# yycho0108/qpwcnet

Hardware: AMD Instinct MI355X
Metric: image-pairs/sec at 256x512 fp32 (higher is better)
Workload: dtype f32; 1 GPU; BASELINE configs[1]: full 6-level PWC-Net (qpwcnet build_flower) inference, batch 8 per GPU, 256x512 fp32, channels_last, d=4 cost volume + WarpV2; global_batch=8, batch_per_gpu=8, parallelism=dp1 (pairs sharded, RCCL all-gather of the 6 per-level EPE), hipgraph=True

## Files before the change

### qpwcnet_amd/csrc/encoder.hip

```cpp
#include "common.h"
#include "launch.h"

namespace qpwc {

__device__ __forceinline__ float enc_mishf(float x) {
    const float e = __builtin_amdgcn_exp2f(fminf(x, 20.0f) * 1.4426950408889634f);
    const float t = e * (e + 2.0f);
    const float m = x * (t * __builtin_amdgcn_rcpf(t + 2.0f));
    return m;
}

typedef float f32x4e __attribute__((ext_vector_type(4)));

__device__ __forceinline__ float2 ld2(const float* p) { return *reinterpret_cast<const float2*>(p); }
__device__ __forceinline__ float2 ld2(const __half* p) { return __half22float2(*reinterpret_cast<const __half2*>(p)); }
__device__ __forceinline__ void st4q(float* p, float4 v) { *reinterpret_cast<float4*>(p) = v; }
__device__ __forceinline__ void st4q(__half* p, float4 v) {
    __half2 lo = __floats2half2_rn(v.x, v.y), hi = __floats2half2_rn(v.z, v.w);
    uint2 u;
    u.x = *reinterpret_cast<unsigned*>(&lo);
    u.y = *reinterpret_cast<unsigned*>(&hi);
    *reinterpret_cast<uint2*>(p) = u;
}

// ... 42 lines not shown
                                                              const float* __restrict__ weight,
                                                              const float* __restrict__ bias,
                                                              float* __restrict__ out, int H, int W,
                                                              int pad_h, int pad_w, int tiles_x, int tiles_y,
                                                              int groups_x) {
    constexpr int NQ = C / 4;
    constexpr int NFT = C / 16;
    constexpr int NKC = C / 16;
    constexpr int NLD = (kEcNH * NQ + 255) / 256;
    constexpr int NBUF = NT > 1 ? 2 : 1;
    __shared__ __attribute__((aligned(16))) float in_s[NBUF * kEcNH * C];
    const int tid0 = threadIdx.x;
    const int wave = __builtin_amdgcn_readfirstlane(tid0 >> 6);
    const int lane = tid0 & 63, n0 = lane & 15, g0 = lane >> 4;
    const int grp = xcd_swizzle(blockIdx.x, gridDim.x);
    const int gx0 = grp % groups_x, ty = (grp / groups_x) % tiles_y, b = grp / (groups_x * tiles_y);
    const int tx0 = gx0 * NT;
    const int Y0 = ty * kEcTH;
    const float* xb = x + (int64_t)b * H * W * C;
    const int Ho = H + pad_h, Wo = W + pad_w;
    float* ob = out + (int64_t)b * Ho * Wo * C;

    auto stage_load = [&](int tid, int tx, float4 (&v)[NLD]) {
        const int X0 = tx * kEcTW;
#pragma unroll
        for (int it = 0; it < NLD; ++it) {
            const int idx = tid + 256 * it;
            const int hp = idx / NQ, q = idx - hp * NQ;
            const int hy = hp / kEcHW, hx = hp - hy * kEcHW;
            const int gy = Y0 - 1 + hy, gx = X0 - 1 + hx;
            v[it] = (idx < kEcNH * NQ && gy >= 0 && gy < H && gx >= 0 && gx < W)
                        ? *reinterpret_cast<const float4*>(xb + ((int64_t)gy * W + gx) * C + 4 * q)
                        : make_float4(0.f, 0.f, 0.f, 0.f);
        }
    };
    auto stage_write = [&](int tid, int buf, const float4 (&v)[NLD]) {
#pragma unroll
        for (int it = 0; it < NLD; ++it) {
            const int idx = tid + 256 * it;
            const int hp = idx / NQ, q = idx - hp * NQ;
            if (idx < kEcNH * NQ)
                *reinterpret_cast<float4*>(in_s + buf * (kEcNH * C) + hp * C + 4 * ec_slot<C>(q, hp)) = v[it];
        }
    };
#ifdef QPWC_ENC_STAMP
    const bool census_on = tid0 == 0 && blockIdx.x < 4096;
    long long* census_p = g_enc_census + (blockIdx.x < 4096 ? blockIdx.x : 0) * 6;
    if (census_on)
        census_p[5] = (long long)(unsigned)__builtin_amdgcn_s_getreg((4) | (0 << 6) | (31 << 11)) |
                      ((long long)(unsigned)__builtin_amdgcn_s_getreg((20) | (0 << 6) | (31 << 11)) << 32);
#endif
    ENC_CENSUS(0);
    float4 st[NLD];
    stage_load(tid0, tx0, st);
#ifdef QPWC_ENC_STAMP
    asm volatile("s_waitcnt vmcnt(0)" ::: "memory");
#endif
    ENC_CENSUS(1);
    stage_write(tid0, 0, st);
    __syncthreads();
    ENC_CENSUS(2);

#pragma unroll 1
    for (int t = 0; t < NT; ++t) {
        const int tx = tx0 + t;
        if (tx >= tiles_x) break;
        const bool more = t + 1 < NT && tx + 1 < tiles_x;

        const int X0 = tx * kEcTW;
        const float* tile_s = in_s + (t & (NBUF - 1)) * (kEcNH * C);
        const float* wt = weight;
        int n = n0, g = g0, tid = tid0;
        if (NT > 1) asm volatile("" : "+r"(wt), "+v"(n), "+v"(g), "+v"(tid));
        if (more) stage_load(tid, tx + 1, st);
#pragma unroll
        for (int ft = 0; ft < NFT; ++ft) {
            f32x4e wld[9][NKC];
#pragma unroll
            for (int k = 0; k < 9; ++k)
#pragma unroll
                for (int kc = 0; kc < NKC; ++kc)
                    wld[k][kc] = *reinterpret_cast<const f32x4e*>(wt + ((int64_t)k * C + 16 * ft + n) * C + 16 * kc + 4 * g);
            f32x4e acc[2];
            acc[0] = f32x4e{0.f, 0.f, 0.f, 0.f};
            acc[1] = f32x4e{0.f, 0.f, 0.f, 0.f};
#pragma unroll
            for (int ky = 0; ky < 3; ++ky)
#pragma unroll
                for (int kx = 0; kx < 3; ++kx)
#pragma unroll
                    for (int kc = 0; kc < NKC; ++kc) {
                        f32x4e bv[2];
#pragma unroll
                        for (int m = 0; m < 2; ++m) {
                            const int hp = (2 * wave + m + ky) * kEcHW + n + kx;
                            const int q = 4 * kc + g;
                            const int slot = ec_slot<C>(q, hp);
                            bv[m] = *reinterpret_cast<const f32x4e*>(tile_s + hp * C + 4 * slot);
                        }
#pragma unroll
                        for (int tt = 0; tt < 4; ++tt)
#pragma unroll
                            for (int m = 0; m < 2; ++m)
                                acc[m] = __builtin_amdgcn_mfma_f32_16x16x4f32(wld[ky * 3 + kx][kc][tt], bv[m][tt], acc[m], 0, 0, 0);
                    }
            if (ft == NFT - 1) ENC_CENSUS(3);
            const float4 bq = *reinterpret_cast<const float4*>(bias + 16 * ft + 4 * g);
#pragma unroll
            for (int m = 0; m < 2; ++m) {
                const int gy = Y0 + 2 * wave + m, gx = X0 + n;
                if (gy < H && gx < W)
                    *reinterpret_cast<float4*>(ob + ((int64_t)gy * Wo + gx) * C + 16 * ft + 4 * g) =
                        make_float4(enc_mishf(acc[m][0] + bq.x), enc_mishf(acc[m][1] + bq.y),
                                    enc_mishf(acc[m][2] + bq.z), enc_mishf(acc[m][3] + bq.w));
            }
        }
        if (pad_w > 0 && X0 + kEcTW >= W) {
            for (int i = tid; i < kEcTH * pad_w * NQ; i += 256) {
                const int q = i % NQ, r = i / NQ, col = r % pad_w, row = r / pad_w;
                const int gy = Y0 + row;
                if (gy < H) *reinterpret_cast<float4*>(ob + ((int64_t)gy * Wo + W + col) * C + 4 * q) = make_float4(0.f, 0.f, 0.f, 0.f);
            }
        }
        if (pad_h > 0 && Y0 + kEcTH >= H) {
            const int x_end = (X0 + kEcTW >= W) ? Wo : X0 + kEcTW;
            for (int i = tid; i < pad_h * (x_end - X0) * NQ; i += 256) {
                const int q = i % NQ, r = i / NQ, col = r % (x_end - X0), row = r / (x_end - X0);
                *reinterpret_cast<float4*>(ob + ((int64_t)(H + row) * Wo + X0 + col) * C + 4 * q) = make_float4(0.f, 0.f, 0.f, 0.f);
            }
        }
        ENC_CENSUS(4);
        if (more) {
            stage_write(tid, (t + 1) & (NBUF - 1), st);
            __syncthreads();
        }
    }
}

constexpr int kEwSlots = 5;
constexpr unsigned kEwOob = 0x80000000u;

template <int C, int TH>
struct EwShape {
    static constexpr int NKB = C / 32;
    static constexpr int NS = 9 * NKB;
    static constexpr int NH = (TH + 2) * kEcHW;
    static constexpr int NHI = (NH * 8 + 255) / 256;
    static constexpr int HBLK = 4 * NHI * 1024;
    static constexpr int WBASE = 2 * HBLK;
    static constexpr int LDS = WBASE + 4 * kEwSlots * 2048;
    static_assert(NKB % 2 == 0, "the K-loop walks pairs of 32-channel blocks");
};

__device__ __forceinline__ void ew_wait_vm(int n) {
    switch (n) {
#define EW_W(k) case k: asm volatile("s_waitcnt vmcnt(" #k ")" ::: "memory"); break;
        EW_W(1) EW_W(2) EW_W(3) EW_W(4) EW_W(5) EW_W(6) EW_W(7) EW_W(8) EW_W(9) EW_W(10) EW_W(11) EW_W(12)
#undef EW_W
        default: asm volatile("s_waitcnt vmcnt(0)" ::: "memory"); break;
    }
}

__device__ __forceinline__ void ew_dma16(__amdgpu_buffer_rsrc_t r, char* lds, unsigned voff, int soff) {
#ifdef __HIP_DEVICE_COMPILE__
    typedef __attribute__((address_space(3))) void* lds_ptr_t;
    __builtin_amdgcn_raw_ptr_buffer_load_lds(r, (lds_ptr_t)lds, 16, voff, soff, 0, 0);
#endif
}

__device__ __forceinline__ void ew_pin_agpr(f32x4e& v) {
#ifdef __HIP_DEVICE_COMPILE__
    asm volatile("" : "+a"(v));
#endif
}

template <int C, int TH>
__global__ __launch_bounds__(256, (2 * EwShape<C, TH>::LDS <= 160 * 1024) ? 2 : 1) void conv3x3_mish_ring_kernel(
    const float* __restrict__ x, const float* __restrict__ weight, const float* __restrict__ bias,
    float* __restrict__ out, int H, int W, int pad_h, int pad_w, int tiles_x, int tiles_y, int n_tiles) {
    using S = EwShape<C, TH>;
    __shared__ __attribute__((aligned(1024))) char smem[S::LDS];
    const int tid = threadIdx.x;
    const int wave = __builtin_amdgcn_readfirstlane(tid >> 6);
    const int lane = tid & 63, n = lane & 15, g = lane >> 4;
    const int slice = blockIdx.x / n_tiles;
    const int tile = xcd_swizzle(blockIdx.x % n_tiles, n_tiles);
    const int tx = tile % tiles_x, ty = (tile / tiles_x) % tiles_y, b = tile / (tiles_x * tiles_y);
    const int X0 = tx * kEcTW, Y0 = ty * TH;
    const int fo = 64 * slice + 16 * wave;
    const __amdgpu_buffer_rsrc_t rx = __builtin_amdgcn_make_buffer_rsrc(
        const_cast<float*>(x) + (int64_t)b * H * W * C, 0, H * W * C * 4, 0x00020000);
    const __amdgpu_buffer_rsrc_t rw = __builtin_amdgcn_make_buffer_rsrc(const_cast<float*>(weight), 0, 9 * C * C * 4, 0x00020000);

    unsigned hoff[S::NHI];
#pragma unroll
    for (int j = 0; j < S::NHI; ++j) {
        const int i = (wave * S::NHI + j) * 64 + lane;
        const int hp = i >> 3, q = (i & 7) ^ (hp & 7);
        const int hy = hp / kEcHW, hx = hp - hy * kEcHW;
        const int gy = Y0 - 1 + hy, gx = X0 - 1 + hx;
        hoff[j] = (hp < S::NH && gy >= 0 && gy < H && gx >= 0 && gx < W) ? (unsigned)(((gy * W + gx) * C + 4 * q) * 4) : kEwOob;
    }
    const unsigned woff = (unsigned)(((fo + n) * C + 4 * g) * 4);
    auto issue_h = [&](int kb) __attribute__((always_inline)) {
#pragma unroll
        for (int j = 0; j < S::NHI; ++j)
            ew_dma16(rx, smem + (kb & 1) * S::HBLK + (wave * S::NHI + j) * 1024, hoff[j], kb * 128);
    };
    auto issue_w = [&](int s) __attribute__((always_inline)) {
        const int sc = s < S::NS ? s : S::NS - 1;
        const int kb = sc / 9, tap = sc - 9 * kb;
        char* dst = smem + S::WBASE + ((s % kEwSlots) * 4 + wave) * 2048;
#pragma unroll
        for (int kc = 0; kc < 2; ++kc)
            ew_dma16(rw, dst + kc * 1024, woff, (tap * C * C + 32 * kb + 16 * kc) * 4);
    };
    f32x4e wa[2][2], pb[2][2][TH];
    auto read = [&](int s, int buf) __attribute__((always_inline)) {
        const int kb = s / 9, tap = s - 9 * kb, ky = tap / 3, kx = tap - 3 * ky;
        const char* ws = smem + S::WBASE + ((s % kEwSlots) * 4 + wave) * 2048 + lane * 16;
        const char* hs = smem + (kb & 1) * S::HBLK;
#pragma unroll
        for (int kc = 0; kc < 2; ++kc) {
            wa[buf][kc] = *reinterpret_cast<const f32x4e*>(ws + kc * 1024);
#pragma unroll
            for (int m = 0; m < TH; ++m) {
                const int hp = (m + ky) * kEcHW + n + kx;
                pb[buf][kc][m] = *reinterpret_cast<const f32x4e*>(hs + hp * 128 + 16 * ((4 * kc + g) ^ (hp & 7)));
            }
        }
    };
    f32x4e acc[TH];
#pragma unroll
    for (int m = 0; m < TH; ++m) {
        acc[m] = f32x4e{0.f, 0.f, 0.f, 0.f};
        ew_pin_agpr(acc[m]);
    }

    issue_h(0);
#pragma unroll
    for (int s = 0; s < kEwSlots - 1; ++s) issue_w(s);
    ew_wait_vm(2 * (kEwSlots - 2));
    __builtin_amdgcn_s_barrier();
    read(0, 0);

    auto pair = [&](int p, const bool LAST) __attribute__((always_inline)) {
#pragma unroll
        for (int t = 0; t < 18; ++t) {
            const int s = 18 * p + t;
            const bool more = !(LAST && t == 17);
            if (more) {
                const int tb = t % 9;
                const bool h_young = tb >= 1 && tb <= kEwSlots - 2 && !(LAST && t >= 9);
                ew_wait_vm(2 * (kEwSlots - 3) + (h_young ? S::NHI : 0));
                if (tb == 8) {
                    asm volatile("s_waitcnt lgkmcnt(0)" ::: "memory");
                    __builtin_amdgcn_s_barrier();
                }
            }
            issue_w(s + kEwSlots - 1);
            if (t == 0) issue_h(2 * p + 1);
            if (t == 9 && !LAST) issue_h(2 * p + 2);
            if (more) read(s + 1, (t + 1) & 1);
            __builtin_amdgcn_sched_barrier(0);
#pragma unroll
            for (int kc = 0; kc < 2; ++kc)
#pragma unroll
                for (int tt = 0; tt < 4; ++tt)
#pragma unroll
                    for (int m = 0; m < TH; ++m)
                        acc[m] = __builtin_amdgcn_mfma_f32_16x16x4f32(wa[t & 1][kc][tt], pb[t & 1][kc][m][tt], acc[m], 0, 0, 0);
#pragma unroll
            for (int m = 0; m < TH; ++m) ew_pin_agpr(acc[m]);
            __builtin_amdgcn_sched_barrier(0);
        }
    };
#pragma unroll 1
    for (int p = 0; p < S::NKB / 2 - 1; ++p) pair(p, false);
    pair(S::NKB / 2 - 1, true);
    asm volatile("s_waitcnt vmcnt(0)" ::: "memory");

    const int Ho = H + pad_h, Wo = W + pad_w;
    float* ob = out + (int64_t)b * Ho * Wo * C;
    const float4 bq = *reinterpret_cast<const float4*>(bias + fo + 4 * g);
#pragma unroll
    for (int m = 0; m < TH; ++m) {
        const int gy = Y0 + m, gx = X0 + n;
        if (gy < H && gx < W)
            *reinterpret_cast<float4*>(ob + ((int64_t)gy * Wo + gx) * C + fo + 4 * g) =
                make_float4(enc_mishf(acc[m][0] + bq.x), enc_mishf(acc[m][1] + bq.y),
                            enc_mishf(acc[m][2] + bq.z), enc_mishf(acc[m][3] + bq.w));
    }
    if (pad_w > 0 && X0 + kEcTW >= W) {
        for (int i = tid; i < TH * pad_w * 16; i += 256) {
            const int q = i & 15, r = i >> 4, col = r % pad_w, row = r / pad_w;
            const int gy = Y0 + row;
            if (gy < H) *reinterpret_cast<float4*>(ob + ((int64_t)gy * Wo + W + col) * C + 64 * slice + 4 * q) = make_float4(0.f, 0.f, 0.f, 0.f);
        }
    }
    if (pad_h > 0 && Y0 + TH >= H) {
        const int x_end = (X0 + kEcTW >= W) ? Wo : X0 + kEcTW;
        for (int i = tid; i < pad_h * (x_end - X0) * 16; i += 256) {
            const int q = i & 15, r = i >> 4, col = r % (x_end - X0), row = r / (x_end - X0);
            *reinterpret_cast<float4*>(ob + ((int64_t)(H + row) * Wo + X0 + col) * C + 64 * slice + 4 * q) = make_float4(0.f, 0.f, 0.f, 0.f);
        }
    }
}

template <int C, int TH>
static int conv3x3_mish_ring_launch(const void* x, const void* weight, const void* bias, void* out, int B, int H,
// ... 712 lines not shown
    } else {
        constexpr int NP = (kFcIH * kFcIW * 3 + 255) / 256;
        float2 pv[NP];
#pragma unroll
        for (int it = 0; it < NP; ++it) {
            const int idx = tid + 256 * it;
            const int row = idx / (kFcIW * 3), e = idx - row * (kFcIW * 3);
            const int gy = 2 * Y0 + row, gx = 2 * X0 + e / 3;
            pv[it] = make_float2(0.f, 0.f);
            if (idx < kFcIH * kFcIW * 3 && gy < H && gx < W) pv[it] = ld2(xb + ((int64_t)gy * W + 2 * X0) * 6 + 2 * e);
        }
#pragma unroll
        for (int it = 0; it < NP; ++it) {
            const int idx = tid + 256 * it;
            const int row = idx / (kFcIW * 3), e = idx - row * (kFcIW * 3);
            if (idx < kFcIH * kFcIW * 3) *reinterpret_cast<float2*>(in_s + row * (kFcIW * 6) + 2 * e) = pv[it];
        }
    }
    float wv[9];
#pragma unroll
    for (int k = 0; k < 9; ++k) wv[k] = weight[(k * 16 + n) * 4 + g];
    const float4 bq = *reinterpret_cast<const float4*>(bias + 4 * g);
    __syncthreads();

    const int f = wave >> 1;
    T* ob = out + (int64_t)(f * B + b) * Ho * Wo * 16;
    f32x4e acc[kFcTR];
#pragma unroll
    for (int r = 0; r < kFcTR; ++r) acc[r] = f32x4e{0.f, 0.f, 0.f, 0.f};
    float vb[2][kFcTR];
    auto read_tap = [&](float (&v)[kFcTR], int k) __attribute__((always_inline)) {
        const int ky = k / 3, kx = k - 3 * ky;
#pragma unroll
        for (int r = 0; r < kFcTR; ++r) {
            const int oy = kFcTR * (wave & 1) + r;
            v[r] = in_s[((2 * oy + ky) * kFcIW + 2 * n + kx) * 6 + 3 * f + (g < 3 ? g : 2)];
        }
    };
    read_tap(vb[0], 0);
#pragma unroll
    for (int k = 0; k < 9; ++k) {
        if (k + 1 < 9) read_tap(vb[(k + 1) & 1], k + 1);
        __builtin_amdgcn_sched_barrier(0);
#pragma unroll
        for (int r = 0; r < kFcTR; ++r)
            acc[r] = __builtin_amdgcn_mfma_f32_16x16x4f32(wv[k], g < 3 ? vb[k & 1][r] : 0.0f, acc[r], 0, 0, 0);
        __builtin_amdgcn_sched_barrier(0);
    }
#pragma unroll
    for (int r = 0; r < kFcTR; ++r) {
        const int gy = Y0 + kFcTR * (wave & 1) + r, gx = X0 + n;
        if (gy < Ho && gx < Wo)
            st4q(ob + ((int64_t)gy * Wo + gx) * 16 + 4 * g,
                 make_float4(enc_mishf(acc[r][0] + bq.x), enc_mishf(acc[r][1] + bq.y), enc_mishf(acc[r][2] + bq.z),
                             enc_mishf(acc[r][3] + bq.w)));
    }
}

int first_conv_mish_launch(const void* x, const void* weight, const void* bias, void* out, int B, int H, int W,
                           int layout, int dtype, hipStream_t s) {
    const int tiles_x = (W / 2 + kEcTW - 1) / kEcTW, tiles_y = (H / 2 + kFcTH - 1) / kFcTH;
    const int64_t nblk = (int64_t)tiles_x * tiles_y * B;
    if (nblk > INT32_MAX) {
        set_error("first_conv_mish: too many tiles");
        return QPWC_E_SHAPE;
    }
    if (dtype == QPWC_F32)
        hipLaunchKernelGGL(first_conv_mish_kernel<float>, dim3((unsigned)nblk), dim3(256), 0, s, (const float*)x,
                           (const float*)weight, (const float*)bias, (float*)out, B, H, W, tiles_x, tiles_y,
                           layout == QPWC_NCHW ? 1 : 0);
    else
        hipLaunchKernelGGL(first_conv_mish_kernel<__half>, dim3((unsigned)nblk), dim3(256), 0, s, (const __half*)x,
                           (const float*)weight, (const float*)bias, (__half*)out, B, H, W, tiles_x, tiles_y,
                           layout == QPWC_NCHW ? 1 : 0);
    return check_launch("first_conv_mish_kernel");
}

constexpr int kS2IH = 2 * kEcTH + 1;
constexpr int kS2PW = kEcTW + 1;

__global__ __launch_bounds__(256, 4) void conv3x3s2_mish_kernel(const float* __restrict__ x,
                                                                const float* __restrict__ weight,
                                                                const float* __restrict__ bias,
                                                                float* __restrict__ out, int H, int W,
                                                                int tiles_x, int tiles_y) {
    constexpr int CI = 16, CO = 32;
    __shared__ __attribute__((aligned(16))) float in_s[2 * kS2IH * kS2PW * CI];
    const int tid = threadIdx.x;
    const int wave = __builtin_amdgcn_readfirstlane(tid >> 6);
    const int lane = tid & 63, n = lane & 15, g = lane >> 4;
    const int tile = xcd_swizzle(blockIdx.x, gridDim.x);
    const int tx = tile % tiles_x, ty = (tile / tiles_x) % tiles_y, b = tile / (tiles_x * tiles_y);
    const int X0 = tx * kEcTW, Y0 = ty * kEcTH;
    const int Hp = H + 1, Wp = W + 1, Ho = H / 2, Wo = W / 2;
    const float* xb = x + (int64_t)b * Hp * Wp * CI;
    for (int idx = tid; idx < kS2IH * 33 * 4; idx += 256) {
        const int q = idx & 3, pxl = idx >> 2;
        const int row = pxl / 33, col = pxl - row * 33;
        const int gy = 2 * Y0 + row, gx = 2 * X0 + col;
        float4 v = make_float4(0.f, 0.f, 0.f, 0.f);
        if (gy < Hp && gx < Wp) v = *reinterpret_cast<const float4*>(xb + ((int64_t)gy * Wp + gx) * CI + 4 * q);
        const int pix = ((col & 1) * kS2IH + row) * kS2PW + (col >> 1);
        *reinterpret_cast<float4*>(in_s + pix * CI + 4 * ec_slot<CI>(q, pix)) = v;
    }
    f32x4e wv[9][2];
#pragma unroll
    for (int k = 0; k < 9; ++k)
#pragma unroll
        for (int ft = 0; ft < 2; ++ft)
            wv[k][ft] = *reinterpret_cast<const f32x4e*>(weight + ((int64_t)k * CO + 16 * ft + n) * CI + 4 * g);
    __syncthreads();

    f32x4e acc[2][2];
#pragma unroll
    for (int m = 0; m < 2; ++m)
#pragma unroll
        for (int ft = 0; ft < 2; ++ft) acc[m][ft] = f32x4e{0.f, 0.f, 0.f, 0.f};
#pragma unroll
    for (int ky = 0; ky < 3; ++ky)
#pragma unroll
        for (int kx = 0; kx < 3; ++kx) {
            f32x4e bv[2];
#pragma unroll
            for (int m = 0; m < 2; ++m) {
                const int row = 2 * (2 * wave + m) + ky;
                const int par = kx & 1, pc = n + (kx >> 1);
                const int pix = (par * kS2IH + row) * kS2PW + pc;
                bv[m] = *reinterpret_cast<const f32x4e*>(in_s + pix * CI + 4 * ec_slot<CI>(g, pix));
            }
#pragma unroll
            for (int t = 0; t < 4; ++t)
#pragma unroll
                for (int m = 0; m < 2; ++m)
#pragma unroll
                    for (int ft = 0; ft < 2; ++ft)
                        acc[m][ft] = __builtin_amdgcn_mfma_f32_16x16x4f32(wv[ky * 3 + kx][ft][t], bv[m][t], acc[m][ft], 0, 0, 0);
        }
    float* ob = out + (int64_t)b * Ho * Wo * CO;
    const float4 bq2[2] = {*reinterpret_cast<const float4*>(bias + 4 * g), *reinterpret_cast<const float4*>(bias + 16 + 4 * g)};
#pragma unroll
    for (int ft = 0; ft < 2; ++ft) {
        const float4 bq = bq2[ft];
#pragma unroll
        for (int m = 0; m < 2; ++m) {
            const int gy = Y0 + 2 * wave + m, gx = X0 + n;
            if (gy < Ho && gx < Wo)
                *reinterpret_cast<float4*>(ob + ((int64_t)gy * Wo + gx) * CO + 16 * ft + 4 * g) =
                    make_float4(enc_mishf(acc[m][ft][0] + bq.x), enc_mishf(acc[m][ft][1] + bq.y),
                                enc_mishf(acc[m][ft][2] + bq.z), enc_mishf(acc[m][ft][3] + bq.w));
        }
    }
}

template <int CI, int TH>
__global__ __launch_bounds__(256, (2 * (2 * TH + 1) * (kEcTW + 1) * CI * 4 > 80 * 1024) ? 1 : 2) void conv3x3s2_mish_wide_kernel(const float* __restrict__ x,
                                                                     const float* __restrict__ weight,
                                                                     const float* __restrict__ bias,
                                                                     float* __restrict__ out, int H, int W,
                                                                     int tiles_x, int tiles_y, int n_tiles) {
    constexpr int CO = 2 * CI, NQ = CI / 4, NKB = CI / 32;
    constexpr int IH = 2 * TH + 1, PW = kEcTW + 1;
    constexpr int NPX = IH * 33;
    constexpr int NST = (NPX * NQ + 255) / 256;
    __shared__ __attribute__((aligned(16))) float in_s[2 * IH * PW * CI];
    const int tid = threadIdx.x;
    const int wave = __builtin_amdgcn_readfirstlane(tid >> 6);
    const int lane = tid & 63, n = lane & 15, g = lane >> 4;
    const int slice = blockIdx.x / n_tiles;
    const int tile = xcd_swizzle(blockIdx.x % n_tiles, n_tiles);
    const int tx = tile % tiles_x, ty = (tile / tiles_x) % tiles_y, b = tile / (tiles_x * tiles_y);
    const int X0 = tx * kEcTW, Y0 = ty * TH;
    const int Hp = H + 1, Wp = W + 1, Ho = H / 2, Wo = W / 2;
    const int fo = 64 * slice + 16 * wave;
    const float* xb = x + (int64_t)b * Hp * Wp * CI;
    auto slot = [](int q, int pix) { return CI == 32 ? (q ^ ((pix >> 1) & 7)) : (q ^ (pix & 15)); };
    constexpr int kChunk = NST;
#pragma unroll
    for (int base = 0; base < NST; base += kChunk) {
        float4 st[kChunk];
#pragma unroll
        for (int i = 0; i < kChunk; ++i) {
            const int idx = tid + 256 * (base + i);
            const int pxl = idx / NQ, q = idx - pxl * NQ;
            const int row = pxl / 33, col = pxl - row * 33;
            const int gy = 2 * Y0 + row, gx = 2 * X0 + col;
            st[i] = (base + i < NST && idx < NPX * NQ && gy < Hp && gx < Wp)
                        ? *reinterpret_cast<const float4*>(xb + ((int64_t)gy * Wp + gx) * CI + 4 * q)
                        : make_float4(0.f, 0.f, 0.f, 0.f);
        }
#pragma unroll
        for (int i = 0; i < kChunk; ++i) {
            const int idx = tid + 256 * (base + i);
            const int pxl = idx / NQ, q = idx - pxl * NQ;
            const int row = pxl / 33, col = pxl - row * 33;
            const int pix = ((col & 1) * IH + row) * PW + (col >> 1);
            if (base + i < NST && idx < NPX * NQ) *reinterpret_cast<float4*>(in_s + pix * CI + 4 * slot(q, pix)) = st[i];
        }
    }
    f32x4e acc[TH];
#pragma unroll
    for (int m = 0; m < TH; ++m) acc[m] = f32x4e{0.f, 0.f, 0.f, 0.f};
    f32x4e wv[9][2], wn[9][2];
    auto load_w = [&](f32x4e (&w)[9][2], int kb) {
#pragma unroll
        for (int k = 0; k < 9; ++k)
#pragma unroll
            for (int kc = 0; kc < 2; ++kc)
                w[k][kc] = *reinterpret_cast<const f32x4e*>(weight + ((int64_t)k * CO + fo + n) * CI + 32 * kb + 16 * kc + 4 * g);
    };
    load_w(wv, 0);
    __syncthreads();
    auto block = [&](f32x4e (&wv)[9][2], int kb) __attribute__((always_inline)) {
#pragma unroll
        for (int ky = 0; ky < 3; ++ky)
#pragma unroll
            for (int kx = 0; kx < 3; ++kx)
#pragma unroll
                for (int kc = 0; kc < 2; ++kc) {
                    f32x4e bv[TH];
#pragma unroll
                    for (int m = 0; m < TH; ++m) {
                        const int pix = ((kx & 1) * IH + 2 * m + ky) * PW + n + (kx >> 1);
                        bv[m] = *reinterpret_cast<const f32x4e*>(in_s + pix * CI + 4 * slot(8 * kb + 4 * kc + g, pix));
                    }
#pragma unroll
                    for (int t = 0; t < 4; ++t)
#pragma unroll
                        for (int m = 0; m < TH; ++m)
                            acc[m] = __builtin_amdgcn_mfma_f32_16x16x4f32(wv[ky * 3 + kx][kc][t], bv[m][t], acc[m], 0, 0, 0);
                }
    };
#if QPWC_W_NEXT_ALWAYS
    {
        int kb = 0;
#pragma unroll 1
        for (; kb + 1 < NKB; kb += 2) {
            load_w(wn, kb + 1);
            __builtin_amdgcn_sched_barrier(0);
            block(wv, kb);
            load_w(wv, kb + 2 < NKB ? kb + 2 : kb);
            __builtin_amdgcn_sched_barrier(0);
            block(wn, kb + 1);
        }
        if (kb < NKB) block(wv, kb);
    }
#else
#pragma unroll 1
    for (int kb = 0; kb < NKB; ++kb) {
        if (kb + 1 < NKB) load_w(wn, kb + 1);
        block(wv, kb);
#pragma unroll
        for (int k = 0; k < 9; ++k)
#pragma unroll
            for (int kc = 0; kc < 2; ++kc) wv[k][kc] = wn[k][kc];
    }
#endif
    float* ob = out + (int64_t)b * Ho * Wo * CO;
    const float4 bq = *reinterpret_cast<const float4*>(bias + fo + 4 * g);
#pragma unroll
    for (int m = 0; m < TH; ++m) {
        const int gy = Y0 + m, gx = X0 + n;
        if (gy < Ho && gx < Wo)
            *reinterpret_cast<float4*>(ob + ((int64_t)gy * Wo + gx) * CO + fo + 4 * g) =
                make_float4(enc_mishf(acc[m][0] + bq.x), enc_mishf(acc[m][1] + bq.y),
                            enc_mishf(acc[m][2] + bq.z), enc_mishf(acc[m][3] + bq.w));
    }
}

template <int CI, int TH>
static int conv3x3s2_mish_wide_launch(const void* x, const void* weight, const void* bias, void* out, int B,
                                      int H, int W, hipStream_t s) {
    const int tiles_x = (W / 2 + kEcTW - 1) / kEcTW, tiles_y = (H / 2 + TH - 1) / TH;
    const int64_t n_tiles = (int64_t)tiles_x * tiles_y * B;
    const int slices = 2 * CI / 64;
    if (n_tiles * slices > INT32_MAX) {
        set_error("conv3x3s2_mish: too many tiles");
        return QPWC_E_SHAPE;
    }
    hipLaunchKernelGGL((conv3x3s2_mish_wide_kernel<CI, TH>), dim3((unsigned)(n_tiles * slices)), dim3(256), 0, s,
                       (const float*)x, (const float*)weight, (const float*)bias, (float*)out, H, W, tiles_x, tiles_y,
                       (int)n_tiles);
    return check_launch("conv3x3s2_mish_wide_kernel");
}

int conv3x3s2_mish_any_launch(const void* x, const void* weight, const void* bias, void* out, int B, int H, int W,
                              int CI, hipStream_t s);

int conv3x3s2_mish_launch(const void* x, const void* weight, const void* bias, void* out, int B, int H, int W,
                          hipStream_t s) {
    const int tiles_x = (W / 2 + kEcTW - 1) / kEcTW, tiles_y = (H / 2 + kEcTH - 1) / kEcTH;
    const int64_t nblk = (int64_t)tiles_x * tiles_y * B;
    if (nblk > INT32_MAX) {
        set_error("conv3x3s2_mish: too many tiles");
        return QPWC_E_SHAPE;
    }
    hipLaunchKernelGGL(conv3x3s2_mish_kernel, dim3((unsigned)nblk), dim3(256), 0, s, (const float*)x,
                       (const float*)weight, (const float*)bias, (float*)out, H, W, tiles_x, tiles_y);
    return check_launch("conv3x3s2_mish_kernel");
}

int conv3x3s2_mish_any_launch(const void* x, const void* weight, const void* bias, void* out, int B, int H, int W,
                              int CI, hipStream_t s) {
    switch (CI) {
        case 16: return conv3x3s2_mish_launch(x, weight, bias, out, B, H, W, s);
        case 32: return conv3x3s2_mish_wide_launch<32, 4>(x, weight, bias, out, B, H, W, s);
        case 64: return conv3x3s2_mish_wide_launch<64, 2>(x, weight, bias, out, B, H, W, s);
        case 128: return conv3x3s2_mish_wide_launch<128, 2>(x, weight, bias, out, B, H, W, s);
        default: set_error("conv3x3s2_mish: C_in=%d not in {16,32,64,128}", CI); return QPWC_E_SHAPE;
    }
}

template <int CI, int TH>
__global__ __launch_bounds__(256) void conv3x3s2_mish_f16_kernel(const __half* __restrict__ x,
                                                                const __half* __restrict__ weight,
                                                                const float* __restrict__ bias,
                                                                __half* __restrict__ out, int H, int W, int tiles_x,
                                                                int tiles_y, int n_tiles) {
    constexpr int CO = 2 * CI;
    constexpr int CP = CI < 32 ? 32 : CI;
    constexpr int NQ = CP / 8, NQG = CI / 8, NKB = CP / 32;
    constexpr int IH = 2 * TH + 1, PW = kEcTW + 1;
    constexpr int NB = CO / 16;
    constexpr int WB = NB < 4 ? NB : 4, WR = 4 / WB;
    constexpr int RW = TH / WR;
    constexpr int NCH = IH * (2 * kEcTW + 1) * NQ;
    constexpr int NST = (NCH + 255) / 256;
    __shared__ __attribute__((aligned(16))) __half in_s[2 * IH * PW * CP];
    const int tid = threadIdx.x;
    const int wave = __builtin_amdgcn_readfirstlane(tid >> 6);
    const int lane = tid & 63, n = lane & 15, g = lane >> 4;
    const int slice = blockIdx.x / n_tiles;
    const int tile = xcd_swizzle(blockIdx.x % n_tiles, n_tiles);
    const int tx = tile % tiles_x, ty = (tile / tiles_x) % tiles_y, b = tile / (tiles_x * tiles_y);
    const int X0 = tx * kEcTW, Y0 = ty * TH;
    const int Hp = H + 1, Wp = W + 1, Ho = H / 2, Wo = W / 2;
    const __half* xb = x + (int64_t)b * Hp * Wp * CI;
    {
        uint4 st[NST];
#pragma unroll
        for (int it = 0; it < NST; ++it) {
            const int idx = tid + 256 * it;
            const int q = idx % NQ, pc = idx / NQ;
            const int row = pc / (2 * kEcTW + 1), col = pc - row * (2 * kEcTW + 1);
            const int gy = 2 * Y0 + row, gx = 2 * X0 + col;
            st[it] = (idx < NCH && q < NQG && gy < Hp && gx < Wp)
                         ? *reinterpret_cast<const uint4*>(xb + ((int64_t)gy * Wp + gx) * CI + 8 * q)
                         : make_uint4(0u, 0u, 0u, 0u);
        }
#pragma unroll
        for (int it = 0; it < NST; ++it) {
            const int idx = tid + 256 * it;
            const int q = idx % NQ, pc = idx / NQ;
            const int row = pc / (2 * kEcTW + 1), col = pc - row * (2 * kEcTW + 1);
            const int hp = ((col & 1) * IH + row) * PW + (col >> 1);
            if (idx < NCH) *reinterpret_cast<uint4*>(in_s + hp * CP + 8 * f16_slot<CP>(q, hp)) = st[it];
        }
    }
    const int blk = WB == 4 ? 4 * slice + wave : (wave % WB);
    const int r0 = WB == 4 ? 0 : (wave / WB) * RW;
    const int fo = 16 * blk;
    f32x4e acc[RW];
#pragma unroll
    for (int r = 0; r < RW; ++r) acc[r] = f32x4e{0.f, 0.f, 0.f, 0.f};
    const bool kvalid = 8 * g < CI;
    f16x8e wv[9], wn[9];
    auto load_w = [&](f16x8e (&w)[9], int kb) {
#pragma unroll
        for (int tap = 0; tap < 9; ++tap) {
            w[tap] = f16x8e{0, 0, 0, 0, 0, 0, 0, 0};
            if (kvalid) w[tap] = *reinterpret_cast<const f16x8e*>(weight + ((int64_t)tap * CO + fo + n) * CI + 32 * kb + 8 * g);
        }
    };
    load_w(wv, 0);
    __syncthreads();
    auto block = [&](f16x8e (&wv)[9], int kb) __attribute__((always_inline)) {
#pragma unroll
        for (int tap = 0; tap < 9; ++tap) {
            const int ky = tap / 3, kx = tap - 3 * ky;
#pragma unroll
            for (int r = 0; r < RW; ++r) {
                const int hp = ((kx & 1) * IH + 2 * (r0 + r) + ky) * PW + n + (kx >> 1);
                const f16x8e bv = *reinterpret_cast<const f16x8e*>(in_s + hp * CP + 8 * f16_slot<CP>(4 * kb + g, hp));
                acc[r] = __builtin_amdgcn_mfma_f32_16x16x32_f16(wv[tap], bv, acc[r], 0, 0, 0);
            }
        }
    };
#if QPWC_W_NEXT_ALWAYS_F16
    {
        int kb = 0;
#pragma unroll 1
        for (; kb + 1 < NKB; kb += 2) {
            load_w(wn, kb + 1);
            __builtin_amdgcn_sched_barrier(0);
            block(wv, kb);
            load_w(wv, kb + 2 < NKB ? kb + 2 : kb);
            __builtin_amdgcn_sched_barrier(0);
            block(wn, kb + 1);
        }
        if (kb < NKB) block(wv, kb);
    }
#else
#pragma unroll 1
    for (int kb = 0; kb < NKB; ++kb) {
        if (kb + 1 < NKB) load_w(wn, kb + 1);
        block(wv, kb);
#pragma unroll
        for (int tap = 0; tap < 9; ++tap) wv[tap] = wn[tap];
    }
#endif
    __half* ob = out + (int64_t)b * Ho * Wo * CO;
    const float4 bq = *reinterpret_cast<const float4*>(bias + fo + 4 * g);
#pragma unroll
    for (int r = 0; r < RW; ++r) {
        const int gy = Y0 + r0 + r, gx = X0 + n;
        if (gy < Ho && gx < Wo)
            st4q(ob + ((int64_t)gy * Wo + gx) * CO + fo + 4 * g,
                 make_float4(enc_mishf(acc[r][0] + bq.x), enc_mishf(acc[r][1] + bq.y), enc_mishf(acc[r][2] + bq.z),
                             enc_mishf(acc[r][3] + bq.w)));
    }
}

template <int CI, int TH>
static int conv3x3s2_mish_f16_launch_t(const void* x, const void* weight, const void* bias, void* out, int B, int H,
                                       int W, hipStream_t s) {
    constexpr int NSL = (2 * CI / 16) < 4 ? 1 : (2 * CI / 16) / 4;
    const int tiles_x = (W / 2 + kEcTW - 1) / kEcTW, tiles_y = (H / 2 + TH - 1) / TH;
    const int64_t n_tiles = (int64_t)tiles_x * tiles_y * B;
    if (n_tiles * NSL > INT32_MAX) {
        set_error("conv3x3s2_mish_f16: too many tiles");
        return QPWC_E_SHAPE;
    }
    hipLaunchKernelGGL((conv3x3s2_mish_f16_kernel<CI, TH>), dim3((unsigned)(n_tiles * NSL)), dim3(256), 0, s,
                       (const __half*)x, (const __half*)weight, (const float*)bias, (__half*)out, H, W, tiles_x,
                       tiles_y, (int)n_tiles);
    return check_launch("conv3x3s2_mish_f16_kernel");
}

int conv3x3s2_mish_f16_launch(const void* x, const void* weight, const void* bias, void* out, int B, int H, int W,
                              int CI, hipStream_t s) {
    switch (CI) {
        case 16: return conv3x3s2_mish_f16_launch_t<16, 8>(x, weight, bias, out, B, H, W, s);
        case 32: return conv3x3s2_mish_f16_launch_t<32, 8>(x, weight, bias, out, B, H, W, s);
        case 64: return conv3x3s2_mish_f16_launch_t<64, 4>(x, weight, bias, out, B, H, W, s);
        case 128: return conv3x3s2_mish_f16_launch_t<128, 2>(x, weight, bias, out, B, H, W, s);
        default: set_error("conv3x3s2_mish_f16: C_in=%d not in {16,32,64,128}", CI); return QPWC_E_SHAPE;
    }
}

int conv3x3_mish_launch(const void* x, const void* weight, const void* bias, void* out, int B, int H, int W,
                        int C, int pad_h, int pad_w, hipStream_t s) {
    const int tiles_x = (W + kEcTW - 1) / kEcTW, tiles_y = (H + kEcTH - 1) / kEcTH;
    constexpr int NT = QPWC_ENC_NT;
    const int groups_x = (tiles_x + NT - 1) / NT;
    const int64_t nblk = (int64_t)groups_x * tiles_y * B;
    if (nblk > INT32_MAX) {
        set_error("conv3x3_mish: too many tiles");
        return QPWC_E_SHAPE;
    }
    const dim3 grid((unsigned)nblk);
    if (C == 16)
// ... 27 lines not shown
```

Measured before the change: 7304 pairs/s.

## Stream strided conv halo and weights through async LDS DMA ring

Rewrites the stride-2 3x3 conv+Mish encoder kernel for C_in 32/64/128. Halo tiles are now loaded one 32-channel block at a time into double-buffered LDS through buffer_load-to-LDS DMA. Per-tap weights stream through a WS-slot LDS ring, using counted vmcnt waits and barriers so loads overlap the MFMA work. This replaces the old approach of loading the whole halo and holding all 9x2 weight vectors per block in registers. It aims to cut register pressure and exposed load latency, at the cost of more barriers, fragile wait-count bookkeeping, and a new per-tile buffer-size limit.

```diff
diff --git a/qpwcnet_amd/csrc/encoder.hip b/qpwcnet_amd/csrc/encoder.hip
--- a/qpwcnet_amd/csrc/encoder.hip
+++ b/qpwcnet_amd/csrc/encoder.hip
@@ -218,10 +218,12 @@
     static_assert(NKB % 2 == 0, "the K-loop walks pairs of 32-channel blocks");
 };
 
+constexpr int kEwMaxWait = 16;
 __device__ __forceinline__ void ew_wait_vm(int n) {
     switch (n) {
 #define EW_W(k) case k: asm volatile("s_waitcnt vmcnt(" #k ")" ::: "memory"); break;
         EW_W(1) EW_W(2) EW_W(3) EW_W(4) EW_W(5) EW_W(6) EW_W(7) EW_W(8) EW_W(9) EW_W(10) EW_W(11) EW_W(12)
+        EW_W(13) EW_W(14) EW_W(15) EW_W(16)
 #undef EW_W
         default: asm volatile("s_waitcnt vmcnt(0)" ::: "memory"); break;
     }
@@ -1240,17 +1242,40 @@
     }
 }
 
-template <int CI, int TH>
-__global__ __launch_bounds__(256, (2 * (2 * TH + 1) * (kEcTW + 1) * CI * 4 > 80 * 1024) ? 1 : 2) void conv3x3s2_mish_wide_kernel(const float* __restrict__ x,
-                                                                     const float* __restrict__ weight,
-                                                                     const float* __restrict__ bias,
-                                                                     float* __restrict__ out, int H, int W,
-                                                                     int tiles_x, int tiles_y, int n_tiles) {
-    constexpr int CO = 2 * CI, NQ = CI / 4, NKB = CI / 32;
-    constexpr int IH = 2 * TH + 1, PW = kEcTW + 1;
-    constexpr int NPX = IH * 33;
-    constexpr int NST = (NPX * NQ + 255) / 256;
-    __shared__ __attribute__((aligned(16))) float in_s[2 * IH * PW * CI];
+#ifndef QPWC_S2R_TH32
+#define QPWC_S2R_TH32 4
+#define QPWC_S2R_WS32 5
+#endif
+#ifndef QPWC_S2R_TH64
+#define QPWC_S2R_TH64 2
+#define QPWC_S2R_WS64 4
+#endif
+#ifndef QPWC_S2R_TH128
+#define QPWC_S2R_TH128 2
+#define QPWC_S2R_WS128 4
+#endif
+template <int CI, int TH, int WS>
+struct S2rShape {
+    static constexpr int NKB = CI / 32;
+    static constexpr int NS = 9 * NKB;
+    static constexpr int IH = 2 * TH + 1, PW = kEcTW + 1;
+    static constexpr int NP = 2 * IH * PW;
+    static constexpr int NHI = (NP * 8 + 255) / 256;
+    static constexpr int HBLK = 4 * NHI * 1024;
+    static constexpr int WBASE = (NKB > 1 ? 2 : 1) * HBLK;
+    static constexpr int LDS = WBASE + 4 * WS * 2048;
+    static_assert(NKB == 1 || NKB % 2 == 0, "the K-loop walks one block or pairs of 32-channel blocks");
+    static_assert(WS >= 4 && WS <= 9, "W(s + 1) must be older than a younger request, and the halo older than the next block's first weights");
+    static_assert(2 * (WS - 2) <= kEwMaxWait && 2 * (WS - 3) + NHI <= kEwMaxWait, "every wait is a counted one");
+};
+
+template <int CI, int TH, int WS>
+__global__ __launch_bounds__(256, (2 * S2rShape<CI, TH, WS>::LDS <= 160 * 1024) ? 2 : 1) void conv3x3s2_mish_ring_kernel(
+    const float* __restrict__ x, const float* __restrict__ weight, const float* __restrict__ bias,
+    float* __restrict__ out, int H, int W, int tiles_x, int tiles_y, int n_tiles) {
+    using S = S2rShape<CI, TH, WS>;
+    constexpr int CO = 2 * CI;
+    __shared__ __attribute__((aligned(1024))) char smem[S::LDS];
     const int tid = threadIdx.x;
     const int wave = __builtin_amdgcn_readfirstlane(tid >> 6);
     const int lane = tid & 63, n = lane & 15, g = lane >> 4;
@@ -1260,89 +1285,103 @@
     const int X0 = tx * kEcTW, Y0 = ty * TH;
     const int Hp = H + 1, Wp = W + 1, Ho = H / 2, Wo = W / 2;
     const int fo = 64 * slice + 16 * wave;
-    const float* xb = x + (int64_t)b * Hp * Wp * CI;
-    auto slot = [](int q, int pix) { return CI == 32 ? (q ^ ((pix >> 1) & 7)) : (q ^ (pix & 15)); };
-    constexpr int kChunk = NST;
-#pragma unroll
-    for (int base = 0; base < NST; base += kChunk) {
-        float4 st[kChunk];
-#pragma unroll
-        for (int i = 0; i < kChunk; ++i) {
-            const int idx = tid + 256 * (base + i);
-            const int pxl = idx / NQ, q = idx - pxl * NQ;
-            const int row = pxl / 33, col = pxl - row * 33;
-            const int gy = 2 * Y0 + row, gx = 2 * X0 + col;
-            st[i] = (base + i < NST && idx < NPX * NQ && gy < Hp && gx < Wp)
-                        ? *reinterpret_cast<const float4*>(xb + ((int64_t)gy * Wp + gx) * CI + 4 * q)
-                        : make_float4(0.f, 0.f, 0.f, 0.f);
-        }
-#pragma unroll
-        for (int i = 0; i < kChunk; ++i) {
-            const int idx = tid + 256 * (base + i);
-            const int pxl = idx / NQ, q = idx - pxl * NQ;
-            const int row = pxl / 33, col = pxl - row * 33;
-            const int pix = ((col & 1) * IH + row) * PW + (col >> 1);
-            if (base + i < NST && idx < NPX * NQ) *reinterpret_cast<float4*>(in_s + pix * CI + 4 * slot(q, pix)) = st[i];
-        }
-    }
+    const int band = Hp - 2 * Y0 < S::IH ? Hp - 2 * Y0 : S::IH;
+    const __amdgpu_buffer_rsrc_t rx = __builtin_amdgcn_make_buffer_rsrc(
+        const_cast<float*>(x) + (((int64_t)b * Hp + 2 * Y0) * Wp + 2 * X0) * CI, 0, (band * Wp - 2 * X0) * CI * 4,
+        0x00020000);
+    const __amdgpu_buffer_rsrc_t rw = __builtin_amdgcn_make_buffer_rsrc(const_cast<float*>(weight), 0, 9 * CO * CI * 4, 0x00020000);
+
+    unsigned hoff[S::NHI];
+#pragma unroll
+    for (int j = 0; j < S::NHI; ++j) {
+        const int i = (wave * S::NHI + j) * 64 + lane;
+        const int p = i >> 3, q = (i & 7) ^ (p & 7);
+        const int par = p / (S::IH * S::PW), r = p - par * (S::IH * S::PW);
+        const int row = r / S::PW, col = 2 * (r - row * S::PW) + par;
+        hoff[j] = (p < S::NP && col < 2 * kEcTW + 1 && 2 * Y0 + row < Hp && 2 * X0 + col < Wp)
+                      ? (unsigned)(((row * Wp + col) * CI + 4 * q) * 4) : kEwOob;
+    }
+    const unsigned woff = (unsigned)(((fo + n) * CI + 4 * g) * 4);
+    auto issue_h = [&](int kb) __attribute__((always_inline)) {
+#pragma unroll
+        for (int j = 0; j < S::NHI; ++j)
+            ew_dma16(rx, smem + (kb & 1) * S::HBLK + (wave * S::NHI + j) * 1024, hoff[j], kb * 128);
+    };
+    auto issue_w = [&](int s) __attribute__((always_inline)) {
+        const int sc = s < S::NS ? s : S::NS - 1;
+        const int kb = sc / 9, tap = sc - 9 * kb;
+        char* dst = smem + S::WBASE + ((s % WS) * 4 + wave) * 2048;
+#pragma unroll
+        for (int kc = 0; kc < 2; ++kc)
+            ew_dma16(rw, dst + kc * 1024, woff, (tap * CO * CI + 32 * kb + 16 * kc) * 4);
+    };
+    f32x4e wa[2][2], pb[2][2][TH];
+    auto read = [&](int s, int buf) __attribute__((always_inline)) {
+        const int kb = s / 9, tap = s - 9 * kb, ky = tap / 3, kx = tap - 3 * ky;
+        const char* ws = smem + S::WBASE + ((s % WS) * 4 + wave) * 2048 + lane * 16;
+        const char* hs = smem + (kb & 1) * S::HBLK;
+#pragma unroll
+        for (int kc = 0; kc < 2; ++kc) {
+            wa[buf][kc] = *reinterpret_cast<const f32x4e*>(ws + kc * 1024);
+#pragma unroll
+            for (int m = 0; m < TH; ++m) {
+                const int pix = ((kx & 1) * S::IH + 2 * m + ky) * S::PW + n + (kx >> 1);
+                pb[buf][kc][m] = *reinterpret_cast<const f32x4e*>(hs + pix * 128 + 16 * ((4 * kc + g) ^ (pix & 7)));
+            }
+        }
+    };
     f32x4e acc[TH];
 #pragma unroll
-    for (int m = 0; m < TH; ++m) acc[m] = f32x4e{0.f, 0.f, 0.f, 0.f};
-    f32x4e wv[9][2], wn[9][2];
-    auto load_w = [&](f32x4e (&w)[9][2], int kb) {
-#pragma unroll
-        for (int k = 0; k < 9; ++k)
+    for (int m = 0; m < TH; ++m) {
+        acc[m] = f32x4e{0.f, 0.f, 0.f, 0.f};
+        ew_pin_agpr(acc[m]);
+    }
+
+    issue_h(0);
+#pragma unroll
+    for (int s = 0; s < WS - 1; ++s) issue_w(s);
+    ew_wait_vm(2 * (WS - 2));
+    __builtin_amdgcn_s_barrier();
+    read(0, 0);
+
+    auto blocks = [&](int kb0, const int NB, const bool LAST) __attribute__((always_inline)) {
+#pragma unroll
+        for (int t = 0; t < 9 * NB; ++t) {
+            const int s = 9 * kb0 + t, tb = t % 9;
+            const bool more = !(LAST && t == 9 * NB - 1);
+            const bool h_next = !(LAST && t / 9 == NB - 1);
+            if (more) {
+                ew_wait_vm(2 * (WS - 3) + (h_next && tb >= 1 && tb <= WS - 2 ? S::NHI : 0));
+                if (tb == 8) {
+                    asm volatile("s_waitcnt lgkmcnt(0)" ::: "memory");
+                    __builtin_amdgcn_s_barrier();
+                }
+            }
+            issue_w(s + WS - 1);
+            if (tb == 0 && h_next) issue_h(kb0 + t / 9 + 1);
+            if (more) read(s + 1, (t + 1) & 1);
+            __builtin_amdgcn_sched_barrier(0);
 #pragma unroll
             for (int kc = 0; kc < 2; ++kc)
-                w[k][kc] = *reinterpret_cast<const f32x4e*>(weight + ((int64_t)k * CO + fo + n) * CI + 32 * kb + 16 * kc + 4 * g);
-    };
-    load_w(wv, 0);
-    __syncthreads();
-    auto block = [&](f32x4e (&wv)[9][2], int kb) __attribute__((always_inline)) {
-#pragma unroll
-        for (int ky = 0; ky < 3; ++ky)
-#pragma unroll
-            for (int kx = 0; kx < 3; ++kx)
-#pragma unroll
-                for (int kc = 0; kc < 2; ++kc) {
-                    f32x4e bv[TH];
-#pragma unroll
-                    for (int m = 0; m < TH; ++m) {
-                        const int pix = ((kx & 1) * IH + 2 * m + ky) * PW + n + (kx >> 1);
-                        bv[m] = *reinterpret_cast<const f32x4e*>(in_s + pix * CI + 4 * slot(8 * kb + 4 * kc + g, pix));
-                    }
-#pragma unroll
-                    for (int t = 0; t < 4; ++t)
-#pragma unroll
-                        for (int m = 0; m < TH; ++m)
-                            acc[m] = __builtin_amdgcn_mfma_f32_16x16x4f32(wv[ky * 3 + kx][kc][t], bv[m][t], acc[m], 0, 0, 0);
-                }
-    };
-#if QPWC_W_NEXT_ALWAYS
-    {
-        int kb = 0;
+#pragma unroll
+                for (int tt = 0; tt < 4; ++tt)
+#pragma unroll
+                    for (int m = 0; m < TH; ++m)
+                        acc[m] = __builtin_amdgcn_mfma_f32_16x16x4f32(wa[t & 1][kc][tt], pb[t & 1][kc][m][tt], acc[m], 0, 0, 0);
+#pragma unroll
+            for (int m = 0; m < TH; ++m) ew_pin_agpr(acc[m]);
+            __builtin_amdgcn_sched_barrier(0);
+        }
+    };
+    if constexpr (S::NKB == 1) {
+        blocks(0, 1, true);
+    } else {
 #pragma unroll 1
-        for (; kb + 1 < NKB; kb += 2) {
-            load_w(wn, kb + 1);
-            __builtin_amdgcn_sched_barrier(0);
-            block(wv, kb);
-            load_w(wv, kb + 2 < NKB ? kb + 2 : kb);
-            __builtin_amdgcn_sched_barrier(0);
-            block(wn, kb + 1);
-        }
-        if (kb < NKB) block(wv, kb);
-    }
-#else
-#pragma unroll 1
-    for (int kb = 0; kb < NKB; ++kb) {
-        if (kb + 1 < NKB) load_w(wn, kb + 1);
-        block(wv, kb);
-#pragma unroll
-        for (int k = 0; k < 9; ++k)
-#pragma unroll
-            for (int kc = 0; kc < 2; ++kc) wv[k][kc] = wn[k][kc];
-    }
-#endif
+        for (int p = 0; p < S::NKB / 2 - 1; ++p) blocks(2 * p, 2, false);
+        blocks(S::NKB - 2, 2, true);
+    }
+    asm volatile("s_waitcnt vmcnt(0)" ::: "memory");
+
     float* ob = out + (int64_t)b * Ho * Wo * CO;
     const float4 bq = *reinterpret_cast<const float4*>(bias + fo + 4 * g);
 #pragma unroll
@@ -1355,8 +1394,8 @@
     }
 }
 
-template <int CI, int TH>
-static int conv3x3s2_mish_wide_launch(const void* x, const void* weight, const void* bias, void* out, int B,
+template <int CI, int TH, int WS>
+static int conv3x3s2_mish_ring_launch(const void* x, const void* weight, const void* bias, void* out, int B,
                                       int H, int W, hipStream_t s) {
     const int tiles_x = (W / 2 + kEcTW - 1) / kEcTW, tiles_y = (H / 2 + TH - 1) / TH;
     const int64_t n_tiles = (int64_t)tiles_x * tiles_y * B;
@@ -1365,7 +1404,11 @@
         set_error("conv3x3s2_mish: too many tiles");
         return QPWC_E_SHAPE;
     }
-    hipLaunchKernelGGL((conv3x3s2_mish_wide_kernel<CI, TH>), dim3((unsigned)(n_tiles * slices)), dim3(256), 0, s,
+    if ((int64_t)(2 * TH + 1) * (W + 1) * CI * 4 > INT32_MAX) {
+        set_error("conv3x3s2_mish: %d input rows of 2 GiB or more", 2 * TH + 1);
+        return QPWC_E_SHAPE;
+    }
+    hipLaunchKernelGGL((conv3x3s2_mish_ring_kernel<CI, TH, WS>), dim3((unsigned)(n_tiles * slices)), dim3(256), 0, s,
                        (const float*)x, (const float*)weight, (const float*)bias, (float*)out, H, W, tiles_x, tiles_y,
                        (int)n_tiles);
     return check_launch("conv3x3s2_mish_wide_kernel");
@@ -1391,9 +1434,9 @@
                               int CI, hipStream_t s) {
     switch (CI) {
         case 16: return conv3x3s2_mish_launch(x, weight, bias, out, B, H, W, s);
-        case 32: return conv3x3s2_mish_wide_launch<32, 4>(x, weight, bias, out, B, H, W, s);
-        case 64: return conv3x3s2_mish_wide_launch<64, 2>(x, weight, bias, out, B, H, W, s);
-        case 128: return conv3x3s2_mish_wide_launch<128, 2>(x, weight, bias, out, B, H, W, s);
+        case 32: return conv3x3s2_mish_ring_launch<32, QPWC_S2R_TH32, QPWC_S2R_WS32>(x, weight, bias, out, B, H, W, s);
+        case 64: return conv3x3s2_mish_ring_launch<64, QPWC_S2R_TH64, QPWC_S2R_WS64>(x, weight, bias, out, B, H, W, s);
+        case 128: return conv3x3s2_mish_ring_launch<128, QPWC_S2R_TH128, QPWC_S2R_WS128>(x, weight, bias, out, B, H, W, s);
         default: set_error("conv3x3s2_mish: C_in=%d not in {16,32,64,128}", CI); return QPWC_E_SHAPE;
     }
 }
```

After: 7364 pairs/s (median of 6 runs). No clear change (+0.8%).
